# aanna0701/face-recognition-pytorch

Measured on AMD Instinct MI355X. Metric: train imgs/sec IR-50-layout ResNet50 + ArcFace/PartialFC head, 112x112, higher is better.
Workload: dtype bf16

## Files before the change

face-recognition-pytorch_amd/frhip/csrc/bn.hip:

```cpp
#include "common.h"
#include "frhip.h"

namespace frhip {

constexpr int EW_THREADS = 256;
constexpr int RED_GROUPS = 16;

template <typename T> struct EW {
    static constexpr int EPV = 16 / (int)sizeof(T);
};

template <typename T, bool BWD, bool RS = false>
__global__ __launch_bounds__(EW_THREADS) void colreduce_kernel(const T* __restrict__ x, const T* __restrict__ y,
                                                               const float* __restrict__ mean, const float* __restrict__ invstd,
                                                               const float* __restrict__ mscale, const float* __restrict__ mshift,
                                                               float* __restrict__ partial, int rows, int C,
                                                               const float* __restrict__ rowscale = nullptr, int rows_per = 1) {
    constexpr int EPV = EW<T>::EPV;
    const int vpr = C / EPV;
    const int cg = threadIdx.x % vpr, rl = threadIdx.x / vpr, rlanes = EW_THREADS / vpr;
    float s1[EPV], s2[EPV], mu[EPV], is[EPV], ms[EPV], mb[EPV];
#pragma unroll
    for (int e = 0; e < EPV; ++e) {
        s1[e] = 0.f; s2[e] = 0.f;
        if (BWD) {
            mu[e] = mean[cg * EPV + e]; is[e] = invstd[cg * EPV + e];
            ms[e] = mscale ? mscale[cg * EPV + e] : 0.f; mb[e] = mscale ? mshift[cg * EPV + e] : 1.f;
        }
    }
    for (int r = blockIdx.x * rlanes + rl; r < rows; r += gridDim.x * rlanes) {
        const size_t idx = (size_t)r * C + cg * EPV;
        const Vec16<T> a = *reinterpret_cast<const Vec16<T>*>(x + idx);
        if (BWD) {
            const Vec16<T> b = *reinterpret_cast<const Vec16<T>*>(y + idx);
            float ks = 1.f;
            if constexpr (RS) ks = rowscale[r / rows_per];
#pragma unroll
            for (int e = 0; e < EPV; ++e) {
                const float yy = b.get(e);
                const float d = (yy * ms[e] + mb[e] > 0.f) ? a.get(e) * ks : 0.f;
                s1[e] += d; s2[e] += d * (yy - mu[e]) * is[e];
            }
        } else {
#pragma unroll
            for (int e = 0; e < EPV; ++e) { const float v = a.get(e); s1[e] += v; s2[e] += v * v; }
        }
    }
    __shared__ float red[2][EW_THREADS][EPV + 1];
#pragma unroll
    for (int e = 0; e < EPV; ++e) { red[0][threadIdx.x][e] = s1[e]; red[1][threadIdx.x][e] = s2[e]; }
    __syncthreads();
    for (int t = threadIdx.x; t < 2 * C; t += EW_THREADS) {
        const int st = t / C, c = t - st * C;
        float acc = 0.f;
        for (int k = 0; k < rlanes; ++k) acc += red[st][k * vpr + c / EPV][c % EPV];
        partial[((size_t)blockIdx.x * 2 + st) * C + c] = acc;
    }
}

constexpr int RP_MAX = 16;
__global__ __launch_bounds__(256) void reduce_partials_kernel(const float* __restrict__ in, float* __restrict__ out, int nparts, int C) {
    __shared__ float red[4][64];
    const int tl = threadIdx.x & 63, pl = threadIdx.x >> 6;
    const int t = blockIdx.x * 64 + tl;
    float acc = 0.f;
    if (t < 2 * C) {
        const int stride = gridDim.y * 4;
        for (int p0 = blockIdx.y * 4 + pl; p0 < nparts; p0 += stride * RP_MAX) {
            float v[RP_MAX];
#pragma unroll
            for (int u = 0; u < RP_MAX; ++u) { const int p = p0 + u * stride; v[u] = p < nparts ? in[(size_t)p * 2 * C + t] : 0.f; }
#pragma unroll
            for (int u = 0; u < RP_MAX; ++u) acc += v[u];
        }
    }
    red[pl][tl] = acc;
    __syncthreads();
    if (pl == 0 && t < 2 * C) out[(size_t)blockIdx.y * 2 * C + t] = red[0][tl] + red[1][tl] + red[2][tl] + red[3][tl];
}

constexpr int FIN_MAX_PL = 16;
__device__ __forceinline__ void sum_parts(const float* __restrict__ parts, int nparts, int C, int c, int pl,
                                          float (*red)[2][64], float& s1, float& s2) {
    const int PL = blockDim.x >> 6;
    float a1 = 0.f, a2 = 0.f;
    if (c < C) {
        int p = pl;
        for (; p + 7 * PL < nparts; p += 8 * PL) {
            float x[8], y[8];
#pragma unroll
            for (int u = 0; u < 8; ++u) { const float* r = parts + (size_t)(p + u * PL) * 2 * C; x[u] = r[c]; y[u] = r[C + c]; }
            a1 += ((x[0] + x[1]) + (x[2] + x[3])) + ((x[4] + x[5]) + (x[6] + x[7]));
            a2 += ((y[0] + y[1]) + (y[2] + y[3])) + ((y[4] + y[5]) + (y[6] + y[7]));
        }
        for (; p + 3 * PL < nparts; p += 4 * PL) {
            const float* r0 = parts + (size_t)p * 2 * C, *r1 = r0 + (size_t)PL * 2 * C, *r2 = r1 + (size_t)PL * 2 * C,
                        *r3 = r2 + (size_t)PL * 2 * C;
            const float x0 = r0[c], y0 = r0[C + c], x1 = r1[c], y1 = r1[C + c], x2 = r2[c], y2 = r2[C + c], x3 = r3[c], y3 = r3[C + c];
            a1 += (x0 + x1) + (x2 + x3); a2 += (y0 + y1) + (y2 + y3);
        }
        for (; p < nparts; p += PL) { a1 += parts[(size_t)p * 2 * C + c]; a2 += parts[(size_t)p * 2 * C + C + c]; }
    }
    red[pl][0][threadIdx.x & 63] = a1; red[pl][1][threadIdx.x & 63] = a2;
    __syncthreads();
    const int cl = threadIdx.x & 63;
    s1 = 0.f; s2 = 0.f;
    for (int l = 0; l < PL; ++l) { s1 += red[l][0][cl]; s2 += red[l][1][cl]; }
}

__device__ __forceinline__ void sum_parts16(const float* __restrict__ parts, int nparts, int C, int c, int pl,
                                            float (*red)[2][16], float& s1, float& s2) {
    float a1 = 0.f, a2 = 0.f;
    if (c < C) {
        int p = pl;
        for (; p + 7 * 16 < nparts; p += 8 * 16) {
            float x[8], y[8];
#pragma unroll
            for (int u = 0; u < 8; ++u) { const float* r = parts + (size_t)(p + u * 16) * 2 * C; x[u] = r[c]; y[u] = r[C + c]; }
            a1 += ((x[0] + x[1]) + (x[2] + x[3])) + ((x[4] + x[5]) + (x[6] + x[7]));
            a2 += ((y[0] + y[1]) + (y[2] + y[3])) + ((y[4] + y[5]) + (y[6] + y[7]));
        }
        for (; p < nparts; p += 16) { a1 += parts[(size_t)p * 2 * C + c]; a2 += parts[(size_t)p * 2 * C + C + c]; }
    }
    red[pl][0][threadIdx.x & 15] = a1; red[pl][1][threadIdx.x & 15] = a2;
    __syncthreads();
    const int cl = threadIdx.x & 15;
    s1 = 0.f; s2 = 0.f;
#pragma unroll
// ... 89 lines not shown
template <typename T, bool NTL, bool RS = false, bool INPLACE = false>
__global__ __launch_bounds__(EW_THREADS) void bn_apply_kernel(const T* __restrict__ y_in, const float* __restrict__ scale,
                                                              const float* __restrict__ shift, const T* __restrict__ res,
                                                              const float* __restrict__ rscale, const float* __restrict__ rshift,
                                                              int relu, T* __restrict__ out, int rows, int C,
                                                              const float* __restrict__ rowscale = nullptr, int rows_per = 1) {
    constexpr int EPV = EW<T>::EPV;
    const int vpr = C / EPV;
    const int cg = threadIdx.x % vpr, rl = threadIdx.x / vpr, rlanes = EW_THREADS / vpr;
    float sc[EPV], sh[EPV], rs[EPV], rb[EPV];
    const T* y = INPLACE ? out : y_in;
#pragma unroll
    for (int e = 0; e < EPV; ++e) {
        sc[e] = scale[cg * EPV + e]; sh[e] = shift[cg * EPV + e];
        rs[e] = rscale ? rscale[cg * EPV + e] : 1.f; rb[e] = rscale ? rshift[cg * EPV + e] : 0.f;
    }
#pragma unroll 2
    for (int r = blockIdx.x * rlanes + rl; r < rows; r += gridDim.x * rlanes) {
        const size_t idx = (size_t)r * C + cg * EPV;
        Vec16<T> a = ew_load<T, NTL>(y + idx);
        if constexpr (RS) {
            const float ks = rowscale[r / rows_per];
            Vec16<T> rv;
            if (res) rv = ew_load<T, NTL>(res + idx);
#pragma unroll
            for (int e = 0; e < EPV; ++e) {
                float o = (a.get(e) * sc[e] + sh[e]) * ks + (res ? rv.get(e) * rs[e] + rb[e] : 0.f);
                a.set(e, relu ? fmaxf(o, 0.f) : o);
            }
        } else if (res) {
            const Vec16<T> rv = ew_load<T, NTL>(res + idx);
#pragma unroll
            for (int e = 0; e < EPV; ++e) {
                float o = a.get(e) * sc[e] + sh[e] + (rv.get(e) * rs[e] + rb[e]);
                a.set(e, relu ? fmaxf(o, 0.f) : o);
            }
        } else {
#pragma unroll
            for (int e = 0; e < EPV; ++e) {
                float o = a.get(e) * sc[e] + sh[e];
                a.set(e, relu ? fmaxf(o, 0.f) : o);
            }
        }
        *reinterpret_cast<Vec16<T>*>(out + idx) = a;
    }
}

template <typename T, bool NTL, bool RS = false>
__global__ __launch_bounds__(EW_THREADS) void bn_bwd_apply_kernel(const T* __restrict__ dout, const T* __restrict__ y,
                                                                  const float* __restrict__ ca, const float* __restrict__ cb,
                                                                  const float* __restrict__ cc, const float* __restrict__ mscale,
                                                                  const float* __restrict__ mshift, T* __restrict__ dy,
                                                                  int rows, int C, const float* __restrict__ rowscale = nullptr,
                                                                  int rows_per = 1) {
    constexpr int EPV = EW<T>::EPV;
    const int vpr = C / EPV;
    const int cg = threadIdx.x % vpr, rl = threadIdx.x / vpr, rlanes = EW_THREADS / vpr;
    float a_[EPV], b_[EPV], c_[EPV], ms[EPV], mb[EPV];
#pragma unroll
    for (int e = 0; e < EPV; ++e) {
        a_[e] = ca[cg * EPV + e]; b_[e] = cb[cg * EPV + e]; c_[e] = cc[cg * EPV + e];
        ms[e] = mscale ? mscale[cg * EPV + e] : 0.f; mb[e] = mscale ? mshift[cg * EPV + e] : 1.f;
    }
#pragma unroll 2
    for (int r = blockIdx.x * rlanes + rl; r < rows; r += gridDim.x * rlanes) {
        const size_t idx = (size_t)r * C + cg * EPV;
        const Vec16<T> d = ew_load<T, NTL>(dout + idx);
        Vec16<T> b = ew_load<T, NTL>(y + idx);
        float ks = 1.f;
        if constexpr (RS) ks = rowscale[r / rows_per];
#pragma unroll
        for (int e = 0; e < EPV; ++e) {
            const float yy = b.get(e);
            const float de = (yy * ms[e] + mb[e] > 0.f) ? d.get(e) * ks : 0.f;
            b.set(e, a_[e] * de + b_[e] * yy + c_[e]);
        }
        *reinterpret_cast<Vec16<T>*>(dy + idx) = b;
    }
}

constexpr int EW_BATCH = 4;
constexpr int EW_ROWS_PER_THREAD = 8;
#define EW_BATCH_REGS __attribute__((amdgpu_num_vgpr(96)))
template <int N> __device__ __forceinline__ void coef_load(float (&dst)[N], const float* __restrict__ src) {
#pragma unroll
    for (int q = 0; q < N / 4; ++q) {
        const f32x4_t v = *reinterpret_cast<const f32x4_t*>(src + 4 * q);
        dst[4 * q] = v[0]; dst[4 * q + 1] = v[1]; dst[4 * q + 2] = v[2]; dst[4 * q + 3] = v[3];
    }
}
template <int N> __device__ __forceinline__ void coef_fill(float (&dst)[N], float v) {
#pragma unroll
    for (int e = 0; e < N; ++e) dst[e] = v;
}

template <typename T, bool NTL, bool RS = false, bool INPLACE = false>
__global__ __launch_bounds__(EW_THREADS) EW_BATCH_REGS void bn_apply_batched_kernel(const T* __restrict__ y_in, const float* __restrict__ scale,
                                                                      const float* __restrict__ shift, const T* __restrict__ res,
                                                                      const float* __restrict__ rscale, const float* __restrict__ rshift,
                                                                      int relu, T* __restrict__ out, int rows, int C, int rows_per_block,
                                                                      const float* __restrict__ rowscale = nullptr, int rows_per = 1) {
    constexpr int EPV = EW<T>::EPV, U = EW_BATCH;
    const int vpr = C / EPV;
    const int cg = threadIdx.x % vpr, rl = threadIdx.x / vpr, rlanes = EW_THREADS / vpr;
    float sc[EPV], sh[EPV], rs[EPV], rb[EPV];
    const T* y = INPLACE ? out : y_in;
    coef_load(sc, scale + cg * EPV); coef_load(sh, shift + cg * EPV);
    if (rscale) { coef_load(rs, rscale + cg * EPV); coef_load(rb, rshift + cg * EPV); }
    else { coef_fill(rs, 1.f); coef_fill(rb, 0.f); }
    const int r0 = blockIdx.x * rows_per_block, r1 = min(rows, r0 + rows_per_block);
    for (int rb0 = r0 + rl; rb0 < r1; rb0 += U * rlanes) {
        Vec16<T> a[U], rv[U];
        float ks[U];
#pragma unroll
        for (int u = 0; u < U; ++u) {
            const int r = min(rb0 + u * rlanes, r1 - 1);
            a[u] = ew_load<T, NTL>(y + (size_t)r * C + cg * EPV);
        }
        if (res) {
#pragma unroll
            for (int u = 0; u < U; ++u) {
                const int r = min(rb0 + u * rlanes, r1 - 1);
                rv[u] = ew_load<T, NTL>(res + (size_t)r * C + cg * EPV);
            }
        }
        if constexpr (RS) {
#pragma unroll
            for (int u = 0; u < U; ++u) ks[u] = rowscale[min(rb0 + u * rlanes, r1 - 1) / rows_per];
        }
#pragma unroll
        for (int u = 0; u < U; ++u) {
            if constexpr (RS) {
#pragma unroll
                for (int e = 0; e < EPV; ++e) {
                    float o = (a[u].get(e) * sc[e] + sh[e]) * ks[u] + (res ? rv[u].get(e) * rs[e] + rb[e] : 0.f);
                    a[u].set(e, relu ? fmaxf(o, 0.f) : o);
                }
            } else if (res) {
#pragma unroll
                for (int e = 0; e < EPV; ++e) {
                    float o = a[u].get(e) * sc[e] + sh[e] + (rv[u].get(e) * rs[e] + rb[e]);
                    a[u].set(e, relu ? fmaxf(o, 0.f) : o);
                }
            } else {
#pragma unroll
                for (int e = 0; e < EPV; ++e) {
                    float o = a[u].get(e) * sc[e] + sh[e];
                    a[u].set(e, relu ? fmaxf(o, 0.f) : o);
                }
            }
        }
#pragma unroll
        for (int u = 0; u < U; ++u) {
            const int r = rb0 + u * rlanes;
            if (r < r1) *reinterpret_cast<Vec16<T>*>(out + (size_t)r * C + cg * EPV) = a[u];
        }
    }
}

template <typename T, bool NTL, bool RS = false>
__global__ __launch_bounds__(EW_THREADS) EW_BATCH_REGS void bn_bwd_apply_batched_kernel(const T* __restrict__ dout, const T* __restrict__ y,
                                                                          const float* __restrict__ ca, const float* __restrict__ cb,
                                                                          const float* __restrict__ cc, const float* __restrict__ mscale,
                                                                          const float* __restrict__ mshift, T* __restrict__ dy,
                                                                          int rows, int C, int rows_per_block,
                                                                          const float* __restrict__ rowscale = nullptr, int rows_per = 1) {
    constexpr int EPV = EW<T>::EPV, U = EW_BATCH;
    const int vpr = C / EPV;
    const int cg = threadIdx.x % vpr, rl = threadIdx.x / vpr, rlanes = EW_THREADS / vpr;
    float a_[EPV], b_[EPV], c_[EPV], ms[EPV], mb[EPV];
    coef_load(a_, ca + cg * EPV); coef_load(b_, cb + cg * EPV); coef_load(c_, cc + cg * EPV);
    if (mscale) { coef_load(ms, mscale + cg * EPV); coef_load(mb, mshift + cg * EPV); }
    else { coef_fill(ms, 0.f); coef_fill(mb, 1.f); }
    const int r0 = blockIdx.x * rows_per_block, r1 = min(rows, r0 + rows_per_block);
    for (int rb0 = r0 + rl; rb0 < r1; rb0 += U * rlanes) {
        Vec16<T> d[U], b[U];
        float ks[U];
// ... 338 lines not shown
```

face-recognition-pytorch_amd/frhip/csrc/head.hip:

```cpp
#include "igemm_nt.h"
#include "margin_shared.h"
#include "frhip.h"

namespace frhip {

struct MarginConstEx : MarginConst { float m3, thr; };

constexpr int MG_ARC = 0, MG_ARC_EASY = 1, MG_COS = 2, MG_ROWS = 3;
struct MarginRows { float s, eps; const float* m_ang; const float* m_add; };
template <int MK, bool FILT> struct MarginArgOf { typedef MarginConstEx type; };
template <> struct MarginArgOf<MG_ARC, false> { typedef MarginConst type; };
template <> struct MarginArgOf<MG_ROWS, false> { typedef MarginRows type; };
template <int MK, bool FILT>
using MarginArg = typename MarginArgOf<MK, FILT>::type;

template <typename T>
__global__ __launch_bounds__(256) void l2norm_rows_kernel(const float* __restrict__ x, T* __restrict__ xhat,
                                                          float* __restrict__ norms, int rows, int D, float eps) {
    const int row = blockIdx.x * 4 + (threadIdx.x >> 6), lane = threadIdx.x & 63;
    if (row >= rows) return;
    const float* xr = x + (size_t)row * D;
    float ss = 0.f;
    for (int j = lane * 4; j < D; j += 256) {
        const f32x4_t v = *reinterpret_cast<const f32x4_t*>(xr + j);
// ... 181 lines not shown
        }
    }
}

template <typename T, bool FWD, int MK, bool FILT>
__global__ __launch_bounds__(256, 2) void head_kernel(NtGeom g, const void* __restrict__ ehat,
                                                             const void* __restrict__ what, const int* __restrict__ labels,
                                                             MarginArg<MK, FILT> mc, float* __restrict__ part_max,
                                                             float* __restrict__ part_sum, float* __restrict__ ztarget,
                                                             const float* __restrict__ rowmax, const float* __restrict__ rowsum,
                                                             float gscale, const float* __restrict__ upstream,
                                                             void* __restrict__ dt, int ldt, void* __restrict__ dtt, int ldtt,
                                                             int mtiles, int ntiles) {
    typedef NtTile<T, 2, 2> Tile;
    extern __shared__ __attribute__((aligned(16))) char smem[];
    const uint32_t lin = xcd_remap(blockIdx.x, gridDim.x);
    const int mtile = (int)(lin % (uint32_t)mtiles), ntile = (int)(lin / (uint32_t)mtiles);
    NtMainloop<T, 2, 2> ml;
    ml.run(g, ehat, what, smem, mtile, ntile, 0, g.ksteps);

    const int lane = lane_id(), wave = wave_id();
    const int wm = wave >> 1, wn = wave & 1;
    const int m0 = mtile * Tile::BM + wm * 64, n0 = ntile * Tile::BN + wn * 64;
    head_epilogue<FWD, MK, FILT, false>(lane, g, ml.acc, nullptr, m0, n0, ntile * 2 + wn, labels, mc, part_max, part_sum, ztarget, nullptr,
                                        rowmax, rowsum, gscale, upstream);
    if (!FWD) head_store_tile<T>(g, ml, smem, m0, n0, reinterpret_cast<T*>(dt), ldt, ldt, reinterpret_cast<T*>(dtt), ldtt);
}

constexpr int HEAD_SUB_MAX = 4;

template <typename T, bool FWD, int MK, bool FILT>
__global__ __launch_bounds__(256, 2) void head_sub_kernel(NtGeom g, const void* __restrict__ ehat,
                                                                 const void* __restrict__ what, const int* __restrict__ labels,
                                                                 MarginArg<MK, FILT> mc, int K, float* __restrict__ part_max,
                                                                 float* __restrict__ part_sum, float* __restrict__ ztarget,
                                                                 int* __restrict__ tsub, const float* __restrict__ rowmax,
                                                                 const float* __restrict__ rowsum, float gscale,
                                                                 const float* __restrict__ upstream, void* __restrict__ dt, int ldt,
                                                                 int ldp, void* __restrict__ dtt, int ldtt, int mtiles, int ntiles) {
    typedef NtTile<T, 2, 2> Tile;
    extern __shared__ __attribute__((aligned(16))) char smem[];
    const uint32_t lin = xcd_remap(blockIdx.x, gridDim.x);
    const int mtile = (int)(lin % (uint32_t)mtiles), ntile = (int)(lin / (uint32_t)mtiles);
    NtMainloop<T, 2, 2> ml;
    f32x4_t best[4][4];
    uint32_t win[4] = {0u, 0u, 0u, 0u};
    for (int k = 0; k < K; ++k) {
        if (k) __syncthreads();
        ml.run(g, ehat, reinterpret_cast<const char*>(what) + (size_t)k * g.b_bytes, smem, mtile, ntile, 0, g.ksteps);
#pragma unroll
        for (int nt = 0; nt < 4; ++nt)
#pragma unroll
            for (int mt = 0; mt < 4; ++mt)
#pragma unroll
                for (int e = 0; e < 4; ++e) {
                    const float v = ml.acc[nt][mt][e];
                    if (k == 0) best[nt][mt][e] = v;
                    else if (v > best[nt][mt][e]) {
                        best[nt][mt][e] = v;
                        win[nt] = (win[nt] & ~(3u << (2 * (4 * mt + e)))) | ((uint32_t)k << (2 * (4 * mt + e)));
                    }
                }
    }

    const int lane = lane_id(), wave = wave_id();
    const int wm = wave >> 1, wn = wave & 1;
    const int m0 = mtile * Tile::BM + wm * 64, n0 = ntile * Tile::BN + wn * 64;
    head_epilogue<FWD, MK, FILT, true>(lane, g, best, win, m0, n0, ntile * 2 + wn, labels, mc, part_max, part_sum, ztarget, tsub, rowmax,
                                       rowsum, gscale, upstream);
    if (!FWD)
        for (int k = 0; k < K; ++k) {
#pragma unroll
            for (int nt = 0; nt < 4; ++nt)
#pragma unroll
                for (int mt = 0; mt < 4; ++mt)
#pragma unroll
                    for (int e = 0; e < 4; ++e)
                        ml.acc[nt][mt][e] = ((win[nt] >> (2 * (4 * mt + e))) & 3u) == (uint32_t)k ? best[nt][mt][e] : 0.f;
            head_store_tile<T>(g, ml, smem, m0, n0, reinterpret_cast<T*>(dt) + (size_t)k * ldp, ldt, ldp,
                               dtt ? reinterpret_cast<T*>(dtt) + (size_t)k * g.Nout * ldtt : nullptr, ldtt);
        }
}

__global__ __launch_bounds__(256) void head_rowreduce_kernel(const float* __restrict__ part_max, const float* __restrict__ part_sum,
                                                             int ngroups, int N, float* __restrict__ rowmax, float* __restrict__ rowsum) {
    __shared__ float smax[16][17], ssum[16][17];
    const int ml = threadIdx.x & 15, gl = threadIdx.x >> 4;
    const int m = blockIdx.x * 16 + ml;
    float mx = -INFINITY, s = 0.f;
    if (m < N) {
        for (int gq = gl; gq < ngroups; gq += 16) {
            const float pm = part_max[(size_t)gq * N + m], ps = part_sum[(size_t)gq * N + m];
            if (pm > mx) { s = s * __expf(mx - pm) + ps; mx = pm; }
            else if (pm > -INFINITY) s += ps * __expf(pm - mx);
        }
    }
    smax[gl][ml] = mx; ssum[gl][ml] = s;
    __syncthreads();
    if (gl == 0 && m < N) {
        float M = -INFINITY;
#pragma unroll
        for (int k = 0; k < 16; ++k) M = fmaxf(M, smax[k][ml]);
        float S = 0.f;
#pragma unroll
        for (int k = 0; k < 16; ++k) if (smax[k][ml] > -INFINITY) S += ssum[k][ml] * __expf(smax[k][ml] - M);
        rowmax[m] = M; rowsum[m] = S;
    }
}

__global__ void head_rescale_kernel(float* __restrict__ rowsum, const float* __restrict__ local_max,
                                    const float* __restrict__ global_max, int N) {
    const int m = blockIdx.x * blockDim.x + threadIdx.x;
    if (m < N) rowsum[m] *= __expf(local_max[m] - global_max[m]);
}

__global__ void head_target_prob_kernel(const float* __restrict__ ztarget, const int* __restrict__ labels,
                                        const float* __restrict__ rowmax, const float* __restrict__ rowsum,
                                        float* __restrict__ q, int N) {
    const int m = blockIdx.x * blockDim.x + threadIdx.x;
    if (m < N) q[m] = labels[m] >= 0 ? __expf(ztarget[m] - rowmax[m]) / rowsum[m] : 0.f;
}

__global__ void head_pack_stats_kernel(const float* __restrict__ ztarget, const int* __restrict__ labels,
                                       const float* __restrict__ rowmax, const float* __restrict__ rowsum,
                                       float* __restrict__ packed, int N) {
    const int m = blockIdx.x * blockDim.x + threadIdx.x;
    if (m < N) {
        packed[3 * m + 0] = rowmax[m];
        packed[3 * m + 1] = rowsum[m];
        packed[3 * m + 2] = labels[m] >= 0 ? ztarget[m] : -INFINITY;
    }
}

__global__ void head_merge_stats_kernel(const float* __restrict__ gathered, int ws, int N, float* __restrict__ gmax,
                                        float* __restrict__ gsum, float* __restrict__ q) {
    const int m = blockIdx.x * blockDim.x + threadIdx.x;
    if (m >= N) return;
    float M = -INFINITY;
    for (int r = 0; r < ws; ++r) M = fmaxf(M, gathered[((size_t)r * N + m) * 3]);
    float S = 0.f, num = 0.f;
    for (int r = 0; r < ws; ++r) {
        const float* g = gathered + ((size_t)r * N + m) * 3;
        S += g[1] * __expf(g[0] - M);
        if (g[2] > -INFINITY) num += __expf(g[2] - M);
    }
    gmax[m] = M; gsum[m] = S; q[m] = num / S;
}

__global__ void head_loss_kernel(const float* __restrict__ q, int N, float* __restrict__ loss) {
    __shared__ float red[256];
    float acc = 0.f;
    for (int m = threadIdx.x; m < N; m += 256) acc += logf(fmaxf(q[m], 1e-30f));
    red[threadIdx.x] = acc;
    __syncthreads();
    for (int d = 128; d > 0; d >>= 1) { if (threadIdx.x < d) red[threadIdx.x] += red[threadIdx.x + d]; __syncthreads(); }
    if (threadIdx.x == 0) loss[0] = -red[0] / (float)N;
}

struct HeadMargin { int mk; bool filt; MarginConstEx ex; MarginRows rows; };

template <int MK, bool FILT>
static MarginArg<MK, FILT> margin_arg(const HeadMargin& hm) {
    if constexpr (MK == MG_ROWS) return hm.rows;
    else return hm.ex;
}

struct HeadArgs {
    const void *ehat, *what;
    const int* labels;
    float *pmax, *psum, *zt;
    int* tsub;
    const float *rmax, *rsum;
    float gscale;
    const float* upstream;
    void* dt;
    int ldt, ldp;
    void* dtt;
// ... 308 lines not shown
```

face-recognition-pytorch_amd/frhip/csrc/misc.hip:

```cpp
#include <stdarg.h>
#include <stdio.h>
#include <atomic>
#include "common.h"
#include "frhip.h"

namespace frhip {

static thread_local char g_err[512] = "";

void set_error(const char* fmt, ...) {
    va_list ap;
    va_start(ap, fmt);
    vsnprintf(g_err, sizeof(g_err), fmt, ap);
    va_end(ap);
}

int check_launch(const char* what) {
    hipError_t e = hipGetLastError();
    if (e != hipSuccess) {
        set_error("%s: launch failed: %s", what, hipGetErrorString(e));
        return FRHIP_ELAUNCH;
    }
    return FRHIP_OK;
}

int set_dynamic_lds(const void* fn, int bytes, const char* who) {
    constexpr int SLOTS = 256;
    static std::atomic<const void*> fns[SLOTS];
    static std::atomic<uint64_t> devs[SLOTS];
    int dev = 0;
    if (hipGetDevice(&dev) != hipSuccess) { (void)hipGetLastError(); dev = -1; }
    const uint64_t bit = (dev >= 0 && dev < 64) ? 1ull << dev : 0;
    int slot = -1;
    const size_t h = (size_t)(((uintptr_t)fn >> 4) * 0x9E3779B97F4A7C15ull >> 32);
    for (int i = 0; i < SLOTS && slot < 0; ++i) {
        const int s = (int)((h + i) % SLOTS);
        const void* cur = nullptr;
        if (fns[s].compare_exchange_strong(cur, fn) || cur == fn) slot = s;
    }
    if (slot >= 0 && bit && (devs[slot].load() & bit)) return FRHIP_OK;
    if (hipFuncSetAttribute(fn, hipFuncAttributeMaxDynamicSharedMemorySize, bytes) != hipSuccess) {
        set_error("%s: cannot raise dynamic LDS to %d bytes", who, bytes);
        return FRHIP_ELAUNCH;
    }
    if (slot >= 0) devs[slot].fetch_or(bit);
    return FRHIP_OK;
}

int device_cu_count() {
    static std::atomic<int> cus[16];
    int dev = 0;
    if (hipGetDevice(&dev) != hipSuccess || dev < 0 || dev >= 16) { (void)hipGetLastError(); return 256; }
    int v = cus[dev].load();
    if (!v) {
        if (hipDeviceGetAttribute(&v, hipDeviceAttributeMultiprocessorCount, dev) != hipSuccess || v <= 0) v = 256;
        cus[dev].store(v);
    }
    return v;
}

template <typename T>
__global__ void pack_wt_kernel(const float* __restrict__ w, T* __restrict__ wt, int K, int RS, int C) {
    __shared__ float tile[32][33];
    const int rs = blockIdx.z, c0 = blockIdx.x * 32, k0 = blockIdx.y * 32;
    for (int j = threadIdx.y; j < 32; j += blockDim.y) {
        const int k = k0 + j, c = c0 + threadIdx.x;
        tile[j][threadIdx.x] = (k < K && c < C) ? w[((size_t)k * RS + rs) * C + c] : 0.f;
    }
    __syncthreads();
    for (int j = threadIdx.y; j < 32; j += blockDim.y) {
        const int c = c0 + j, k = k0 + threadIdx.x;
        if (c < C && k < K) wt[((size_t)c * RS + rs) * K + k] = from_f32<T>(tile[threadIdx.x][j]);
    }
}

template <typename T>
__global__ void prep_weights_kernel(const frhip_wprep* __restrict__ tab, int ntensors) {
    __shared__ float tile[32][33];
    int lo = 0, hi = ntensors - 1;
    while (lo < hi) {
        const int mid = (lo + hi + 1) >> 1;
        if (tab[mid].tile_begin <= (int)blockIdx.x) lo = mid; else hi = mid - 1;
    }
    const frhip_wprep e = tab[lo];
    const int K = e.k, RS = e.rs, C = e.c;
    const int ct = (C + 31) >> 5, kt = (K + 31) >> 5;
    int t = (int)blockIdx.x - e.tile_begin;
    const int cti = t % ct; t /= ct;
    const int kti = t % kt; const int rs = t / kt;
    const int c0 = cti * 32, k0 = kti * 32;
    const float* __restrict__ w = e.w;
    T* __restrict__ wc = reinterpret_cast<T*>(e.wc);
    T* __restrict__ wt = reinterpret_cast<T*>(e.wt);
    for (int j = threadIdx.y; j < 32; j += blockDim.y) {
        const int k = k0 + j, c = c0 + threadIdx.x;
        float v = 0.f;
        if (k < K && c < C) {
            const size_t idx = ((size_t)k * RS + rs) * C + c;
            v = w[idx];
            if (wc) wc[idx] = from_f32<T>(v);
        }
        tile[j][threadIdx.x] = v;
    }
    __syncthreads();
    if (wt)
        for (int j = threadIdx.y; j < 32; j += blockDim.y) {
            const int c = c0 + j, k = k0 + threadIdx.x;
            if (c < C && k < K) wt[((size_t)c * RS + rs) * K + k] = from_f32<T>(tile[threadIdx.x][j]);
        }
}

template <typename TI, typename TO>
__global__ void transpose2d_kernel(const TI* __restrict__ in, TO* __restrict__ out, int rows, int cols, int ld_out) {
    __shared__ float tile[32][33];
    const int c0 = blockIdx.x * 32, r0 = blockIdx.y * 32;
    for (int j = threadIdx.y; j < 32; j += blockDim.y) {
        const int r = r0 + j, c = c0 + threadIdx.x;
        tile[j][threadIdx.x] = (r < rows && c < cols) ? to_f32<TI>(in[(size_t)r * cols + c]) : 0.f;
    }
    __syncthreads();
    for (int j = threadIdx.y; j < 32; j += blockDim.y) {
        const int c = c0 + j, r = r0 + threadIdx.x;
        if (c < cols && r < ld_out) out[(size_t)c * ld_out + r] = from_f32<TO>(tile[threadIdx.x][j]);
    }
}

template <typename T>
__global__ void pack_stem_kernel(const float* __restrict__ w, T* __restrict__ wp, int K, int kin, int kp) {
    const int i = blockIdx.x * blockDim.x + threadIdx.x;
    if (i >= K * kp) return;
    const int k = i / kp, j = i - k * kp;
    wp[i] = from_f32<T>(j < kin ? w[k * kin + j] : 0.f);
}
__global__ void unpack_stem_grad_kernel(const float* __restrict__ dwp, float* __restrict__ dw, int K, int kin, int kp) {
    const int i = blockIdx.x * blockDim.x + threadIdx.x;
    if (i >= K * kin) return;
    const int k = i / kin, j = i - k * kin;
    dw[i] += dwp[k * kp + j];
}

template <typename T>
__global__ __launch_bounds__(256) void fc_permute_kernel(const float* __restrict__ w, T* __restrict__ wp, int C, int HW) {
    extern __shared__ float sh[];
    const int n = blockIdx.x, c0 = blockIdx.y * 64;
    const size_t row = (size_t)n * C * HW;
    for (int i = threadIdx.x; i < 64 * HW; i += 256) sh[i] = w[row + (size_t)c0 * HW + i];
    __syncthreads();
    for (int i = threadIdx.x; i < 64 * HW; i += 256) {
        const int p = i / 64, c = i - p * 64;
        wp[row + (size_t)p * C + c0 + c] = from_f32<T>(sh[c * HW + p]);
    }
}
__global__ __launch_bounds__(256) void fc_unpermute_grad_kernel(const float* __restrict__ dwp, float* __restrict__ dw, int C, int HW) {
    extern __shared__ float sh[];
    const int n = blockIdx.x, c0 = blockIdx.y * 64;
    const size_t row = (size_t)n * C * HW;
    for (int i = threadIdx.x; i < 64 * HW; i += 256) {
        const int p = i / 64, c = i - p * 64;
        sh[i] = dwp[row + (size_t)p * C + c0 + c];
    }
    __syncthreads();
    for (int i = threadIdx.x; i < 64 * HW; i += 256) {
        const int c = i / HW, p = i - c * HW;
        dw[row + (size_t)c0 * HW + i] += sh[p * 64 + c];
    }
}

__global__ void gather_rows_kernel(const float* __restrict__ src, const int64_t* __restrict__ index,
                                   float* __restrict__ dst, int n, int D) {
    const int vpr = D / 4;
    for (size_t t = (size_t)blockIdx.x * blockDim.x + threadIdx.x; t < (size_t)n * vpr; t += (size_t)gridDim.x * blockDim.x) {
        const int i = (int)(t / vpr), v = (int)(t - (size_t)i * vpr);
        reinterpret_cast<f32x4_t*>(dst)[t] = reinterpret_cast<const f32x4_t*>(src)[(size_t)index[i] * vpr + v];
    }
}
__global__ void scatter_rows_kernel(const float* __restrict__ src, const int64_t* __restrict__ index,
                                    float* __restrict__ dst, int n, int D) {
    const int vpr = D / 4;
    for (size_t t = (size_t)blockIdx.x * blockDim.x + threadIdx.x; t < (size_t)n * vpr; t += (size_t)gridDim.x * blockDim.x) {
        const int i = (int)(t / vpr), v = (int)(t - (size_t)i * vpr);
        reinterpret_cast<f32x4_t*>(dst)[(size_t)index[i] * vpr + v] = reinterpret_cast<const f32x4_t*>(src)[t];
    }
}

}

using namespace frhip;

extern "C" const char* frhip_last_error(void) { return g_err; }
extern "C" int frhip_abi_version(void) { return 1; }

extern "C" int frhip_pack_wt(int dtype, const float* w, void* wt, int k, int rs, int c, hipStream_t stream) {
    return by_dtype(dtype, "frhip_pack_wt", [&](auto t) {
        typedef decltype(t) T;
        dim3 grid((c + 31) / 32, (k + 31) / 32, rs), block(32, 8);
        hipLaunchKernelGGL(pack_wt_kernel<T>, grid, block, 0, stream, w, (T*)wt, k, rs, c);
        return check_launch("frhip_pack_wt");
    });
}

extern "C" int frhip_prep_conv_weights(int dtype, const frhip_wprep* table, int ntensors, int ntiles, hipStream_t stream) {
    return by_dtype(dtype, "frhip_prep_conv_weights", [&](auto t) {
        typedef decltype(t) T;
        if (!table || ntensors < 1 || ntiles < 1) { set_error("frhip_prep_conv_weights: empty table"); return FRHIP_EINVAL; }
        dim3 block(32, 8);
        hipLaunchKernelGGL(prep_weights_kernel<T>, dim3(ntiles), block, 0, stream, table, ntensors);
        return check_launch("frhip_prep_conv_weights");
    });
}

extern "C" int frhip_transpose2d(int dtype_in, int dtype_out, const void* in, void* out, int rows, int cols, int ld_out, hipStream_t stream) {
    if (ld_out < rows) { set_error("frhip_transpose2d: ld_out %d < rows %d", ld_out, rows); return FRHIP_EINVAL; }
    dim3 grid((cols + 31) / 32, (ld_out + 31) / 32), block(32, 8);
    const int key = dtype_in * 2 + dtype_out;
    switch (key) {
        case 0: hipLaunchKernelGGL((transpose2d_kernel<bf16_t, bf16_t>), grid, block, 0, stream, (const bf16_t*)in, (bf16_t*)out, rows, cols, ld_out); break;
        case 1: hipLaunchKernelGGL((transpose2d_kernel<bf16_t, float>), grid, block, 0, stream, (const bf16_t*)in, (float*)out, rows, cols, ld_out); break;
        case 2: hipLaunchKernelGGL((transpose2d_kernel<float, bf16_t>), grid, block, 0, stream, (const float*)in, (bf16_t*)out, rows, cols, ld_out); break;
        case 3: hipLaunchKernelGGL((transpose2d_kernel<float, float>), grid, block, 0, stream, (const float*)in, (float*)out, rows, cols, ld_out); break;
        default: set_error("frhip_transpose2d: bad dtypes"); return FRHIP_EINVAL;
    }
    return check_launch("frhip_transpose2d");
}

extern "C" int frhip_pack_stem(int dtype, const float* w, void* wp, int k, int kin, int kp, hipStream_t stream) {
    return by_dtype(dtype, "frhip_pack_stem", [&](auto t) {
        typedef decltype(t) T;
        const int n = k * kp;
        hipLaunchKernelGGL(pack_stem_kernel<T>, dim3((n + 255) / 256), dim3(256), 0, stream, w, (T*)wp, k, kin, kp);
        return check_launch("frhip_pack_stem");
    });
}

extern "C" int frhip_unpack_stem_grad(const float* dwp, float* dw, int k, int kin, int kp, hipStream_t stream) {
    const int n = k * kin;
    hipLaunchKernelGGL(unpack_stem_grad_kernel, dim3((n + 255) / 256), dim3(256), 0, stream, dwp, dw, k, kin, kp);
    return check_launch("frhip_unpack_stem_grad");
}

extern "C" int frhip_fc_permute(int dtype, const float* w, void* wp, int nout, int c, int hw, hipStream_t stream) {
    return by_dtype(dtype, "frhip_fc_permute", [&](auto t) {
        typedef decltype(t) T;
        if (c % 64) { set_error("frhip_fc_permute: channels must be a multiple of 64"); return FRHIP_EINVAL; }
        dim3 grid(nout, c / 64);
        const int lds = 64 * hw * 4;
        hipLaunchKernelGGL(fc_permute_kernel<T>, grid, dim3(256), lds, stream, w, (T*)wp, c, hw);
        return check_launch("frhip_fc_permute");
    });
}

extern "C" int frhip_fc_unpermute_grad(const float* dwp, float* dw, int nout, int c, int hw, hipStream_t stream) {
    if (c % 64) { set_error("frhip_fc_unpermute_grad: channels must be a multiple of 64"); return FRHIP_EINVAL; }
    hipLaunchKernelGGL(fc_unpermute_grad_kernel, dim3(nout, c / 64), dim3(256), 64 * hw * 4, stream, dwp, dw, c, hw);
    return check_launch("frhip_fc_unpermute_grad");
}

extern "C" int frhip_gather_rows(const float* src, const int64_t* index, float* dst, int n, int d, hipStream_t stream) {
    if (d % 4) { set_error("frhip_gather_rows: row length must be a multiple of 4"); return FRHIP_EINVAL; }
    if (n == 0) return FRHIP_OK;
    size_t total = (size_t)n * (d / 4); int blocks = (int)((total + 255) / 256); if (blocks > 4096) blocks = 4096;
    hipLaunchKernelGGL(gather_rows_kernel, dim3(blocks), dim3(256), 0, stream, src, index, dst, n, d);
    return check_launch("frhip_gather_rows");
}

extern "C" int frhip_scatter_rows(const float* src, const int64_t* index, float* dst, int n, int d, hipStream_t stream) {
    if (d % 4) { set_error("frhip_scatter_rows: row length must be a multiple of 4"); return FRHIP_EINVAL; }
    if (n == 0) return FRHIP_OK;
    size_t total = (size_t)n * (d / 4); int blocks = (int)((total + 255) / 256); if (blocks > 4096) blocks = 4096;
    hipLaunchKernelGGL(scatter_rows_kernel, dim3(blocks), dim3(256), 0, stream, src, index, dst, n, d);
    return check_launch("frhip_scatter_rows");
}

__global__ void spin_kernel(long long ticks) {
    const long long t0 = wall_clock64();
    while (wall_clock64() - t0 < ticks) __builtin_amdgcn_s_sleep(32);
}
extern "C" int frhip_spin(long long ticks, hipStream_t stream) {
    if (ticks < 0 || ticks > 100000000LL) { frhip::set_error("frhip_spin: ticks out of range"); return FRHIP_EINVAL; }
    hipLaunchKernelGGL(spin_kernel, dim3(1), dim3(64), 0, stream, ticks);
    return frhip::check_launch("frhip_spin");
}
```

face-recognition-pytorch_amd/frhip/ops.py:

```python
import math
import weakref

import ctypes

import torch

from . import _abi
from ._abi import DT_BF16, DT_F32, check, lib

_DT = {torch.bfloat16: DT_BF16, torch.float32: DT_F32}


def dt_of(t):
    return _DT[t.dtype]


def epv(dtype):
    return 8 if dtype == torch.bfloat16 else 4


def _s():
    return torch._C._cuda_getCurrentRawStream(torch.cuda.current_device())


# ... 477 lines not shown
    nb = lib().frhip_stem_blocks(b, h, w)
    coef = stem_bwd_coef(x, wp, dpool, arg, st, gamma, dgamma, dbeta, scratch, part)
    slabs = torch.empty((nb, 64, 32), dtype=torch.float32, device=dev)
    if gram is not None and pooled is not None:
        check(lib().frhip_stem_bwd_wgrad_gram(dt_of(wp), _p(x), _p(wp), _p(dpool), _p(pooled), _p(arg), _p(gram), _p(coef[0]), _p(coef[1]),
                                              _p(coef[2]), b, h, w, _p(slabs), _p(dw27), _s()), "frhip_stem_bwd_wgrad_gram")
        return coef
    check(lib().frhip_stem_bwd_wgrad(dt_of(wp), _p(x), _p(wp), _p(dpool), _p(arg), _p(coef[0]), _p(coef[1]), _p(coef[2]),
                                     _p(st.scale), _p(st.shift), b, h, w, _p(slabs), _p(dw27), _s()), "frhip_stem_bwd_wgrad")
    return coef


def _need_cuda(who, **tensors):
    for name, t in tensors.items():
        if not isinstance(t, torch.Tensor) or not t.is_cuda:
            raise ValueError("%s: %s must be a tensor on the GPU" % (who, name))
        if not t.is_contiguous():
            raise ValueError("%s: %s must be contiguous" % (who, name))


def stem_dx(x, wp, dpool, arg, pooled, coef, eval_mode=False):
    _need_cuda("stem_dx", x=x, wp=wp, dpool=dpool, arg=arg, pooled=pooled, coef=coef)
    if x.dim() != 4 or x.shape[1] != 3 or x.dtype != torch.float32:
        raise ValueError("stem_dx: x must be fp32 [B,3,H,W], got %s %s" % (tuple(x.shape), x.dtype))
    b, _, h, w = x.shape
    pshape = (b, (h - 1) // 2 + 1, (w - 1) // 2 + 1, 64)
    if wp.dtype not in _DT or tuple(wp.shape) != (64, 1, 1, 32):
        raise ValueError("stem_dx: wp must be pack_stem(w, dtype, kp=32) [64,1,1,32], got %s %s" % (tuple(wp.shape), wp.dtype))
    for name, t, dt in (("dpool", dpool, wp.dtype), ("pooled", pooled, wp.dtype), ("arg", arg, torch.uint8)):
        if tuple(t.shape) != pshape or t.dtype != dt:
            raise ValueError("stem_dx: %s must be %s %s, got %s %s" % (name, pshape, dt, tuple(t.shape), t.dtype))
    if tuple(coef.shape) != (3, 64) or coef.dtype != torch.float32:
        raise ValueError("stem_dx: coef must be fp32 [3,64]")
    dx = torch.empty((b, 3, h, w), dtype=torch.float32, device=x.device)
    cb, cc = (None, None) if eval_mode else (coef[1], coef[2])
    check(lib().frhip_stem_dx(dt_of(wp), _p(x), _p(wp), _p(dpool), _p(arg), _p(pooled), _p(coef[0]), _p(cb), _p(cc), b, h, w, _p(dx),
                              _s()), "frhip_stem_dx")
    return dx


def stem_dx_s2(dy0, wp, h, w):
    _need_cuda("stem_dx_s2", dy0=dy0, wp=wp)
    if dy0.dim() != 4 or dy0.dtype not in _DT:
        raise ValueError("stem_dx_s2: dy0 must be [B,Ho,Wo,64] bf16 / fp32")
    b = dy0.shape[0]
    if tuple(dy0.shape) != (b, (h - 1) // 2 + 1, (w - 1) // 2 + 1, 64):
        raise ValueError("stem_dx_s2: dy0 %s does not match a %d x %d image" % (tuple(dy0.shape), h, w))
    if wp.dtype != dy0.dtype or wp.dim() != 4 or wp.shape[0] != 64 or wp.shape[3] < 27 or wp.shape[1] * wp.shape[2] != 1:
        raise ValueError("stem_dx_s2: wp must be pack_stem(w, dtype) [64,1,1,kp] in dy0's dtype")
    dx = torch.empty((b, 3, h, w), dtype=torch.float32, device=dy0.device)
    check(lib().frhip_stem_dx_s2(dt_of(dy0), _p(dy0), _p(wp), wp.shape[3], b, h, w, _p(dx), _s()), "frhip_stem_dx_s2")
    return dx


def pack_wt(w_f32, dtype, out=None):
    k, r, s, c = w_f32.shape
    out = torch.empty((c, r, s, k), dtype=dtype, device=w_f32.device) if out is None else out
    check(lib().frhip_pack_wt(_DT[dtype], _p(w_f32), _p(out), k, r * s, c, _s()), "frhip_pack_wt")
    return out


_WPREP = {}


def prep_conv_weights(weights, dtype):
    import numpy as np
    key = (tuple(w.data_ptr() for w in weights), dtype)
    hit = _WPREP.get(key)
    if hit is None:
        dev = weights[0].device
        total = sum(w.numel() for w in weights)
        arena = torch.empty(2 * total, dtype=dtype, device=dev)
        es = arena.element_size()
        dt = np.dtype([("w", "<u8"), ("wc", "<u8"), ("wt", "<u8"), ("k", "<i4"), ("rs", "<i4"), ("c", "<i4"), ("tile_begin", "<i4")])
        tab = np.empty(len(weights), dtype=dt)
        outs, off, tiles = [], 0, 0
        for i, w in enumerate(weights):
            assert w.is_cuda and w.dtype == torch.float32 and w.is_contiguous()
            k, r, s, c = w.shape
            n = w.numel()
            wc = arena[off:off + n].view(k, r, s, c)
            wt = arena[off + n:off + 2 * n].view(c, r, s, k)
            tab[i] = (w.data_ptr(), wc.data_ptr(), wt.data_ptr(), k, r * s, c, tiles)
            tiles += ((k + 31) // 32) * ((c + 31) // 32) * r * s
            off += 2 * n
            outs.append((wc, wt))
        assert off * es == arena.numel() * es
        table = torch.from_numpy(tab.view(np.uint8).copy()).to(dev)
        if len(_WPREP) >= 8:
            _WPREP.clear()
        hit = _WPREP[key] = (table, len(weights), tiles, outs, arena, list(weights))
    table, n, tiles, outs, _, _ = hit
    check(lib().frhip_prep_conv_weights(_DT[dtype], _p(table), n, tiles, _s()), "frhip_prep_conv_weights")
    return outs


def transpose2d(x, out_dtype=None, out=None, pad_to=1):
    rows, cols = x.shape
    out_dtype = x.dtype if out_dtype is None else out_dtype
    ld = (rows + pad_to - 1) // pad_to * pad_to
    out = torch.empty((cols, ld), dtype=out_dtype, device=x.device) if out is None else out
    check(lib().frhip_transpose2d(dt_of(x), _DT[out_dtype], _p(x), _p(out), rows, cols, out.shape[1], _s()),
          "frhip_transpose2d")
    return out


def pack_stem(w_f32_k27, dtype, kp=None):
    k = w_f32_k27.shape[0]
    if kp is None:
        kp = 64 if dtype == torch.bfloat16 else 32
    out = torch.empty((k, 1, 1, kp), dtype=dtype, device=w_f32_k27.device)
    check(lib().frhip_pack_stem(_DT[dtype], _p(w_f32_k27), _p(out), k, 27, kp, _s()), "frhip_pack_stem")
    return out


def unpack_stem_grad(dwp, dw):
    k, kp = dwp.shape[0], dwp.numel() // dwp.shape[0]
    check(lib().frhip_unpack_stem_grad(_p(dwp), _p(dw), k, 27, kp, _s()), "frhip_unpack_stem_grad")


def fc_permute(w_f32, c, hw, dtype):
    nout = w_f32.shape[0]
    out = torch.empty((nout, hw * c), dtype=dtype, device=w_f32.device)
    check(lib().frhip_fc_permute(_DT[dtype], _p(w_f32), _p(out), nout, c, hw, _s()), "frhip_fc_permute")
    return out


def fc_unpermute_grad(dwp, dw, c, hw):
    check(lib().frhip_fc_unpermute_grad(_p(dwp), _p(dw), dw.shape[0], c, hw, _s()), "frhip_fc_unpermute_grad")


def gather_rows(src, index, out=None):
    n, d = index.numel(), src.shape[1]
    out = torch.empty((n, d), dtype=torch.float32, device=src.device) if out is None else out
    check(lib().frhip_gather_rows(_p(src), _p(index), _p(out), n, d, _s()), "frhip_gather_rows")
    return out


def scatter_rows(src, index, dst):
    check(lib().frhip_scatter_rows(_p(src), _p(index), _p(dst), index.numel(), src.shape[1], _s()), "frhip_scatter_rows")
    return dst


def l2norm_rows(x, dtype, eps=1e-12):
    rows, d = x.shape
    xh = torch.empty((rows, d), dtype=dtype, device=x.device)
    norms = torch.empty((rows,), dtype=torch.float32, device=x.device)
    check(lib().frhip_l2norm_rows(_DT[dtype], _p(x), _p(xh), _p(norms), rows, d, eps, _s()), "frhip_l2norm_rows")
    return xh, norms


def l2norm_bwd(dxhat, xhat, norms, out_scale=1.0):
    rows, d = dxhat.shape
    dx = torch.empty((rows, d), dtype=torch.float32, device=dxhat.device)
    check(lib().frhip_l2norm_bwd(dt_of(xhat), _p(dxhat), _p(xhat), _p(norms), _p(dx), rows, d, out_scale, _s()),
          "frhip_l2norm_bwd")
    return dx


def head_dw(dt, ehat, what, wnorm, out_scale=1.0):
    n, d = ehat.shape
    classes = what.shape[0]
    if not lib().frhip_head_dw_ok(dt_of(ehat), n, classes, d):
        return None
    dw = torch.empty((classes, d), dtype=torch.float32, device=ehat.device)
    check(lib().frhip_head_dw(dt_of(ehat), _p(dt), dt.shape[1], _p(ehat), _p(what), _p(wnorm), _p(dw), n, classes, d, out_scale, _s()),
          "frhip_head_dw")
# ... 488 lines not shown
```

Baseline: 22700.

## Batch loads in BN column reduce and head row reduce; vectorize 64x64 transposes

The BN column-reduce kernel now issues four rows of loads before consuming them, with asm barriers that keep the loads grouped, so more memory requests are in flight. The head row-reduce does the same over eight partial groups. Weight-prep and transpose2d switch from 32x32 scalar tiles to 64x64 tiles with 16-byte vectorized loads and stores, and the prep kernel finds its tensor with a block-wide count instead of a binary search. In exchange the kernels use more registers and shared memory, and the Python tile count must stay in step with the new tile size.

```diff
diff --git a/face-recognition-pytorch_amd/frhip/csrc/bn.hip b/face-recognition-pytorch_amd/frhip/csrc/bn.hip
--- a/face-recognition-pytorch_amd/frhip/csrc/bn.hip
+++ b/face-recognition-pytorch_amd/frhip/csrc/bn.hip
@@ -10,6 +10,19 @@
     static constexpr int EPV = 16 / (int)sizeof(T);
 };
 
+template <int N> __device__ __forceinline__ void coef_load(float (&dst)[N], const float* __restrict__ src) {
+#pragma unroll
+    for (int q = 0; q < N / 4; ++q) {
+        const f32x4_t v = *reinterpret_cast<const f32x4_t*>(src + 4 * q);
+        dst[4 * q] = v[0]; dst[4 * q + 1] = v[1]; dst[4 * q + 2] = v[2]; dst[4 * q + 3] = v[3];
+    }
+}
+template <int N> __device__ __forceinline__ void coef_fill(float (&dst)[N], float v) {
+#pragma unroll
+    for (int e = 0; e < N; ++e) dst[e] = v;
+}
+
+constexpr int CR_BATCH = 4;
 template <typename T, bool BWD, bool RS = false>
 __global__ __launch_bounds__(EW_THREADS) void colreduce_kernel(const T* __restrict__ x, const T* __restrict__ y,
                                                                const float* __restrict__ mean, const float* __restrict__ invstd,
@@ -20,30 +33,45 @@
     const int vpr = C / EPV;
     const int cg = threadIdx.x % vpr, rl = threadIdx.x / vpr, rlanes = EW_THREADS / vpr;
     float s1[EPV], s2[EPV], mu[EPV], is[EPV], ms[EPV], mb[EPV];
-#pragma unroll
-    for (int e = 0; e < EPV; ++e) {
-        s1[e] = 0.f; s2[e] = 0.f;
-        if (BWD) {
-            mu[e] = mean[cg * EPV + e]; is[e] = invstd[cg * EPV + e];
-            ms[e] = mscale ? mscale[cg * EPV + e] : 0.f; mb[e] = mscale ? mshift[cg * EPV + e] : 1.f;
-        }
-    }
-    for (int r = blockIdx.x * rlanes + rl; r < rows; r += gridDim.x * rlanes) {
-        const size_t idx = (size_t)r * C + cg * EPV;
-        const Vec16<T> a = *reinterpret_cast<const Vec16<T>*>(x + idx);
-        if (BWD) {
-            const Vec16<T> b = *reinterpret_cast<const Vec16<T>*>(y + idx);
-            float ks = 1.f;
-            if constexpr (RS) ks = rowscale[r / rows_per];
-#pragma unroll
-            for (int e = 0; e < EPV; ++e) {
-                const float yy = b.get(e);
-                const float d = (yy * ms[e] + mb[e] > 0.f) ? a.get(e) * ks : 0.f;
-                s1[e] += d; s2[e] += d * (yy - mu[e]) * is[e];
+    coef_fill(s1, 0.f); coef_fill(s2, 0.f);
+    if (BWD) {
+        coef_load(mu, mean + cg * EPV); coef_load(is, invstd + cg * EPV);
+        if (mscale) { coef_load(ms, mscale + cg * EPV); coef_load(mb, mshift + cg * EPV); }
+        else { coef_fill(ms, 0.f); coef_fill(mb, 1.f); }
+    }
+    const int stride = gridDim.x * rlanes;
+    for (int r0 = blockIdx.x * rlanes + rl; r0 < rows; r0 += CR_BATCH * stride) {
+        Vec16<T> a[CR_BATCH], b[CR_BATCH];
+        float ks[CR_BATCH];
+#pragma unroll
+        for (int u = 0; u < CR_BATCH; ++u) {
+            const int r = min(r0 + u * stride, rows - 1);
+            const size_t idx = (size_t)r * C + cg * EPV;
+            a[u] = *reinterpret_cast<const Vec16<T>*>(x + idx);
+            if (BWD) b[u] = *reinterpret_cast<const Vec16<T>*>(y + idx);
+            ks[u] = 1.f;
+            if constexpr (RS) ks[u] = rowscale[r / rows_per];
+        }
+#pragma unroll
+        for (int u = 0; u < CR_BATCH; ++u) {
+            asm volatile("" : "+v"(a[u].v));
+            if (BWD) asm volatile("" : "+v"(b[u].v));
+            if (RS) asm volatile("" : "+v"(ks[u]));
+        }
+#pragma unroll
+        for (int u = 0; u < CR_BATCH; ++u) {
+            if (r0 + u * stride >= rows) break;
+            if (BWD) {
+#pragma unroll
+                for (int e = 0; e < EPV; ++e) {
+                    const float yy = b[u].get(e);
+                    const float d = (yy * ms[e] + mb[e] > 0.f) ? a[u].get(e) * ks[u] : 0.f;
+                    s1[e] += d; s2[e] += d * (yy - mu[e]) * is[e];
+                }
+            } else {
+#pragma unroll
+                for (int e = 0; e < EPV; ++e) { const float v = a[u].get(e); s1[e] += v; s2[e] += v * v; }
             }
-        } else {
-#pragma unroll
-            for (int e = 0; e < EPV; ++e) { const float v = a.get(e); s1[e] += v; s2[e] += v * v; }
         }
     }
     __shared__ float red[2][EW_THREADS][EPV + 1];
@@ -299,17 +327,6 @@
 constexpr int EW_BATCH = 4;
 constexpr int EW_ROWS_PER_THREAD = 8;
 #define EW_BATCH_REGS __attribute__((amdgpu_num_vgpr(96)))
-template <int N> __device__ __forceinline__ void coef_load(float (&dst)[N], const float* __restrict__ src) {
-#pragma unroll
-    for (int q = 0; q < N / 4; ++q) {
-        const f32x4_t v = *reinterpret_cast<const f32x4_t*>(src + 4 * q);
-        dst[4 * q] = v[0]; dst[4 * q + 1] = v[1]; dst[4 * q + 2] = v[2]; dst[4 * q + 3] = v[3];
-    }
-}
-template <int N> __device__ __forceinline__ void coef_fill(float (&dst)[N], float v) {
-#pragma unroll
-    for (int e = 0; e < N; ++e) dst[e] = v;
-}
 
 template <typename T, bool NTL, bool RS = false, bool INPLACE = false>
 __global__ __launch_bounds__(EW_THREADS) EW_BATCH_REGS void bn_apply_batched_kernel(const T* __restrict__ y_in, const float* __restrict__ scale,
diff --git a/face-recognition-pytorch_amd/frhip/csrc/head.hip b/face-recognition-pytorch_amd/frhip/csrc/head.hip
--- a/face-recognition-pytorch_amd/frhip/csrc/head.hip
+++ b/face-recognition-pytorch_amd/frhip/csrc/head.hip
@@ -287,6 +287,7 @@
         }
 }
 
+constexpr int RR_BATCH = 8;
 __global__ __launch_bounds__(256) void head_rowreduce_kernel(const float* __restrict__ part_max, const float* __restrict__ part_sum,
                                                              int ngroups, int N, float* __restrict__ rowmax, float* __restrict__ rowsum) {
     __shared__ float smax[16][17], ssum[16][17];
@@ -294,10 +295,19 @@
     const int m = blockIdx.x * 16 + ml;
     float mx = -INFINITY, s = 0.f;
     if (m < N) {
-        for (int gq = gl; gq < ngroups; gq += 16) {
-            const float pm = part_max[(size_t)gq * N + m], ps = part_sum[(size_t)gq * N + m];
-            if (pm > mx) { s = s * __expf(mx - pm) + ps; mx = pm; }
-            else if (pm > -INFINITY) s += ps * __expf(pm - mx);
+        for (int g0 = gl; g0 < ngroups; g0 += 16 * RR_BATCH) {
+            float pm[RR_BATCH], ps[RR_BATCH];
+#pragma unroll
+            for (int u = 0; u < RR_BATCH; ++u) {
+                const int gq = g0 + 16 * u;
+                pm[u] = gq < ngroups ? part_max[(size_t)gq * N + m] : -INFINITY;
+                ps[u] = gq < ngroups ? part_sum[(size_t)gq * N + m] : 0.f;
+            }
+#pragma unroll
+            for (int u = 0; u < RR_BATCH; ++u) {
+                if (pm[u] > mx) { s = s * __expf(mx - pm[u]) + ps[u]; mx = pm[u]; }
+                else if (pm[u] > -INFINITY) s += ps[u] * __expf(pm[u] - mx);
+            }
         }
     }
     smax[gl][ml] = mx; ssum[gl][ml] = s;
diff --git a/face-recognition-pytorch_amd/frhip/csrc/misc.hip b/face-recognition-pytorch_amd/frhip/csrc/misc.hip
--- a/face-recognition-pytorch_amd/frhip/csrc/misc.hip
+++ b/face-recognition-pytorch_amd/frhip/csrc/misc.hip
@@ -74,55 +74,95 @@
     }
 }
 
+constexpr int TB = 64;
+typedef float Tile64[TB][TB + 1];
+#define GLOBAL_AS __attribute__((address_space(1)))
+template <typename T> __device__ __forceinline__ GLOBAL_AS T* as_global(T* p) { return (GLOBAL_AS T*)p; }
+__device__ __forceinline__ bool aligned16(const void* p) { return ((uintptr_t)p & 15) == 0; }
+
+template <typename TI>
+__device__ __forceinline__ void tile_load(Tile64& tile, const GLOBAL_AS TI* __restrict__ src, size_t ld, int nr, int nc, bool vec) {
+    constexpr int EPI = 16 / (int)sizeof(TI), VPR = TB / EPI, NV = TB * VPR / 256;
+    if (nr <= 0 || nc <= 0) {
+        for (int i = threadIdx.x; i < TB * TB; i += 256) tile[i / TB][i % TB] = 0.f;
+    } else if (vec) {
+        Vec16<TI> v[NV];
+#pragma unroll
+        for (int q = 0; q < NV; ++q) {
+            const int i = (int)threadIdx.x + q * 256, r = min(i / VPR, nr - 1), c = min((i % VPR) * EPI, nc - EPI);
+            v[q].v = *reinterpret_cast<const GLOBAL_AS decltype(v[q].v)*>(src + (size_t)r * ld + c);
+        }
+#pragma unroll
+        for (int q = 0; q < NV; ++q) {
+            const int i = (int)threadIdx.x + q * 256, r = i / VPR, c = (i % VPR) * EPI;
+            const bool in = r < nr && c < nc;
+#pragma unroll
+            for (int e = 0; e < EPI; ++e) tile[r][c + e] = in ? v[q].get(e) : 0.f;
+        }
+    } else {
+        for (int i = threadIdx.x; i < TB * TB; i += 256) {
+            const int r = i / TB, c = i % TB;
+            tile[r][c] = (r < nr && c < nc) ? to_f32<TI>(src[(size_t)r * ld + c]) : 0.f;
+        }
+    }
+}
+template <typename TO, bool TRANS>
+__device__ __forceinline__ void tile_store(const Tile64& tile, GLOBAL_AS TO* __restrict__ dst, size_t ld, int ni, int nj, bool vec) {
+    constexpr int EPO = 16 / (int)sizeof(TO), VPR = TB / EPO, NV = TB * VPR / 256;
+    if (vec) {
+#pragma unroll
+        for (int q = 0; q < NV; ++q) {
+            const int t = (int)threadIdx.x + q * 256, i = t / VPR, j = (t % VPR) * EPO;
+            if (i < ni && j < nj) {
+                Vec16<TO> o;
+#pragma unroll
+                for (int e = 0; e < EPO; ++e) o.set(e, TRANS ? tile[j + e][i] : tile[i][j + e]);
+                *reinterpret_cast<GLOBAL_AS decltype(o.v)*>(dst + (size_t)i * ld + j) = o.v;
+            }
+        }
+    } else {
+        for (int t = threadIdx.x; t < TB * TB; t += 256) {
+            const int i = t / TB, j = t % TB;
+            if (i < ni && j < nj) dst[(size_t)i * ld + j] = from_f32<TO>(TRANS ? tile[j][i] : tile[i][j]);
+        }
+    }
+}
+
 template <typename T>
-__global__ void prep_weights_kernel(const frhip_wprep* __restrict__ tab, int ntensors) {
-    __shared__ float tile[32][33];
-    int lo = 0, hi = ntensors - 1;
-    while (lo < hi) {
-        const int mid = (lo + hi + 1) >> 1;
-        if (tab[mid].tile_begin <= (int)blockIdx.x) lo = mid; else hi = mid - 1;
-    }
-    const frhip_wprep e = tab[lo];
+__global__ __launch_bounds__(256) void prep_weights_kernel(const frhip_wprep* __restrict__ tab, int ntensors) {
+    __shared__ Tile64 tile;
+    int below = 0;
+    for (int t0 = 0; t0 < ntensors; t0 += 256) {
+        const int t = t0 + (int)threadIdx.x;
+        below += __syncthreads_count(t < ntensors && tab[t].tile_begin <= (int)blockIdx.x);
+    }
+    const frhip_wprep e = tab[max(below, 1) - 1];
     const int K = e.k, RS = e.rs, C = e.c;
-    const int ct = (C + 31) >> 5, kt = (K + 31) >> 5;
+    const int ct = (C + TB - 1) / TB, kt = (K + TB - 1) / TB;
     int t = (int)blockIdx.x - e.tile_begin;
     const int cti = t % ct; t /= ct;
     const int kti = t % kt; const int rs = t / kt;
-    const int c0 = cti * 32, k0 = kti * 32;
-    const float* __restrict__ w = e.w;
-    T* __restrict__ wc = reinterpret_cast<T*>(e.wc);
-    T* __restrict__ wt = reinterpret_cast<T*>(e.wt);
-    for (int j = threadIdx.y; j < 32; j += blockDim.y) {
-        const int k = k0 + j, c = c0 + threadIdx.x;
-        float v = 0.f;
-        if (k < K && c < C) {
-            const size_t idx = ((size_t)k * RS + rs) * C + c;
-            v = w[idx];
-            if (wc) wc[idx] = from_f32<T>(v);
-        }
-        tile[j][threadIdx.x] = v;
-    }
-    __syncthreads();
-    if (wt)
-        for (int j = threadIdx.y; j < 32; j += blockDim.y) {
-            const int c = c0 + j, k = k0 + threadIdx.x;
-            if (c < C && k < K) wt[((size_t)c * RS + rs) * K + k] = from_f32<T>(tile[threadIdx.x][j]);
-        }
+    if (rs >= RS) return;
+    const int c0 = cti * TB, k0 = kti * TB, nk = min(TB, K - k0), nc = min(TB, C - c0);
+    constexpr int EPO = 16 / (int)sizeof(T);
+    T* wc = reinterpret_cast<T*>(e.wc);
+    T* wt = reinterpret_cast<T*>(e.wt);
+    const size_t at = ((size_t)k0 * RS + rs) * C + c0;
+    tile_load<float>(tile, as_global(e.w) + at, (size_t)RS * C, nk, nc, C % 4 == 0 && aligned16(e.w));
+    __syncthreads();
+    if (wc) tile_store<T, false>(tile, as_global(wc) + at, (size_t)RS * C, nk, nc, C % EPO == 0 && aligned16(wc));
+    if (wt) tile_store<T, true>(tile, as_global(wt) + ((size_t)c0 * RS + rs) * K + k0, (size_t)RS * K, nc, nk, K % EPO == 0 && aligned16(wt));
 }
 
 template <typename TI, typename TO>
-__global__ void transpose2d_kernel(const TI* __restrict__ in, TO* __restrict__ out, int rows, int cols, int ld_out) {
-    __shared__ float tile[32][33];
-    const int c0 = blockIdx.x * 32, r0 = blockIdx.y * 32;
-    for (int j = threadIdx.y; j < 32; j += blockDim.y) {
-        const int r = r0 + j, c = c0 + threadIdx.x;
-        tile[j][threadIdx.x] = (r < rows && c < cols) ? to_f32<TI>(in[(size_t)r * cols + c]) : 0.f;
-    }
-    __syncthreads();
-    for (int j = threadIdx.y; j < 32; j += blockDim.y) {
-        const int c = c0 + j, r = r0 + threadIdx.x;
-        if (c < cols && r < ld_out) out[(size_t)c * ld_out + r] = from_f32<TO>(tile[threadIdx.x][j]);
-    }
+__global__ __launch_bounds__(256) void transpose2d_kernel(const TI* __restrict__ in, TO* __restrict__ out, int rows, int cols, int ld_out) {
+    __shared__ Tile64 tile;
+    constexpr int EPI = 16 / (int)sizeof(TI), EPO = 16 / (int)sizeof(TO);
+    const int c0 = blockIdx.x * TB, r0 = blockIdx.y * TB;
+    tile_load<TI>(tile, as_global(in) + (size_t)r0 * cols + c0, (size_t)cols, min(TB, rows - r0), min(TB, cols - c0), cols % EPI == 0 && aligned16(in));
+    __syncthreads();
+    tile_store<TO, true>(tile, as_global(out) + (size_t)c0 * ld_out + r0, (size_t)ld_out, min(TB, cols - c0), min(TB, ld_out - r0),
+                         ld_out % EPO == 0 && aligned16(out));
 }
 
 template <typename T>
@@ -203,15 +243,14 @@
     return by_dtype(dtype, "frhip_prep_conv_weights", [&](auto t) {
         typedef decltype(t) T;
         if (!table || ntensors < 1 || ntiles < 1) { set_error("frhip_prep_conv_weights: empty table"); return FRHIP_EINVAL; }
-        dim3 block(32, 8);
-        hipLaunchKernelGGL(prep_weights_kernel<T>, dim3(ntiles), block, 0, stream, table, ntensors);
+        hipLaunchKernelGGL(prep_weights_kernel<T>, dim3(ntiles), dim3(256), 0, stream, table, ntensors);
         return check_launch("frhip_prep_conv_weights");
     });
 }
 
 extern "C" int frhip_transpose2d(int dtype_in, int dtype_out, const void* in, void* out, int rows, int cols, int ld_out, hipStream_t stream) {
     if (ld_out < rows) { set_error("frhip_transpose2d: ld_out %d < rows %d", ld_out, rows); return FRHIP_EINVAL; }
-    dim3 grid((cols + 31) / 32, (ld_out + 31) / 32), block(32, 8);
+    dim3 grid((cols + TB - 1) / TB, (ld_out + TB - 1) / TB), block(256);
     const int key = dtype_in * 2 + dtype_out;
     switch (key) {
         case 0: hipLaunchKernelGGL((transpose2d_kernel<bf16_t, bf16_t>), grid, block, 0, stream, (const bf16_t*)in, (bf16_t*)out, rows, cols, ld_out); break;
diff --git a/face-recognition-pytorch_amd/frhip/ops.py b/face-recognition-pytorch_amd/frhip/ops.py
--- a/face-recognition-pytorch_amd/frhip/ops.py
+++ b/face-recognition-pytorch_amd/frhip/ops.py
@@ -583,7 +583,7 @@
             wc = arena[off:off + n].view(k, r, s, c)
             wt = arena[off + n:off + 2 * n].view(c, r, s, k)
             tab[i] = (w.data_ptr(), wc.data_ptr(), wt.data_ptr(), k, r * s, c, tiles)
-            tiles += ((k + 31) // 32) * ((c + 31) // 32) * r * s
+            tiles += ((k + 63) // 64) * ((c + 63) // 64) * r * s
             off += 2 * n
             outs.append((wc, wt))
         assert off * es == arena.numel() * es
```

After: 22790 (median of 6 runs). No clear change (+0.4%).
